# JosefAlbers/Phi-3-Vision-MLX

Measured on AMD Instinct MI355X. Metric: decode tokens/sec through generate()'s loop (reference-defined; bare graph replays: device_rate) + prefill ms, Phi-3-Vision bf16 1-image VQA, higher is better.
Workload: dtype bf16; 1 GPU; Phi-3-Vision single 336x336 image VQA (BASELINE configs[1]); 17 crops, 2509 image tokens + 22 text tokens, prompt 2531, B=1 per GPU, greedy, EOS suppressed; parallelism=batch-sharded replicas x1, batch_per_gpu=1, tiny=False

## Files before the change

include/p3v.h:

```cpp
#ifndef P3V_H
#define P3V_H
#include <stdint.h>

#ifdef __cplusplus
extern "C" {
#endif

#define P3V_VERSION 600
#define P3V_OK 0
#define P3V_ERR_ARG (-22)
#define P3V_ERR_LAUNCH (-5)
#define P3V_ERR_UNSUPPORTED (-95)
#define P3V_ERR_HIP (-14)

typedef struct {
  int cu_count, lds_per_cu, wave_size, clock_khz, mem_clock_khz, mem_bus_bits;
  int64_t hbm_bytes;
  char arch[32];
} p3v_props_t;

int p3v_version(void);
int p3v_device_props(int device, p3v_props_t* out );
const char* p3v_strerror(int code);

// ... 152 lines not shown
                 int h_crops, int w_crops, int grid , int C, void* stream);

int p3v_argmax(const uint16_t* logits, int32_t* out, int rows, int n, int64_t row_stride, void* stream);
int p3v_log_softmax(const uint16_t* x, uint16_t* y, int rows, int n, void* stream);
int p3v_topk(const uint16_t* x, int32_t* idx_out, int rows, int n, int k, int64_t row_stride, void* stream);

typedef struct {
  const uint16_t* x; const uint32_t* W; const uint32_t* sb; void* out;
  const uint16_t* resid; const uint16_t* norm_w; float norm_eps;
  int M, N, K;
  int epilogue;
} p3v_gemv_q4_args_t;
int p3v_gemv_q4(const p3v_gemv_q4_args_t* args , void* stream);
int p3v_dequant_q4(const uint32_t* w4, const uint32_t* sb, uint16_t* out_bf16, int rows, int K, void* stream);

int p3v_resample_u8(const uint8_t* in, uint8_t* out, int outer, int in_len, int out_len, int inner,
                    const int32_t* coeffs, const int32_t* bounds, int ksize, void* stream);
int p3v_hd_preprocess(const uint8_t* resized, int rh, int rw, int top, int hp, int portrait, const double* lut,
                      const float* hw, const int32_t* hi, const float* ww, const int32_t* wi, float* pixel_values,
                      int n_slots, void* stream);

int p3v_lora_down(const uint16_t* x, const float* lora_a, float* t, int M, int K, int r, void* stream);
int p3v_lora_up(const uint16_t* y, const float* t, const float* lora_b, float scale, int epilogue,
                const uint16_t* resid, uint16_t* out, int M, int N, int r, void* stream);

#define P3V_LORA_SLICE_K 256
typedef struct {
  const float* lora_a;
  const float* lora_b;
  int32_t rank;
// ... 15 lines not shown
                   int n_zero, void* stream);
int p3v_step_end(const uint16_t* logits, int32_t* next_tok, int32_t* tok, int32_t* history, int32_t* d_step,
                 int32_t* d_past, int32_t* ticket, int B, int n, int max_steps, void* stream);

#define P3V_GEMV_STEP_MAX_WG 1024
#define P3V_GEMV_STEP_WS_BYTES (P3V_GEMV_STEP_MAX_WG * 8 + 9 * 128)
typedef struct {
  const int32_t* tok; const uint16_t* embed_table; int vocab; uint16_t* x_out;
  const float* cos_t; const float* sin_t; float* cos_out; float* sin_out; int tab_t, half_dim;
  int32_t* next_tok; int32_t* tok_out; int32_t* history; int32_t* d_step; int32_t* ticket; float* amax_ws; int max_steps;
  int32_t* d_past;
} p3v_gemv_step_t;
int p3v_gemv_step(const p3v_gemv_args_t* args , const p3v_gemv_step_t* step , void* stream);
int p3v_gemv_fp8_step(const p3v_gemv_fp8_args_t* args , const p3v_gemv_step_t* step , void* stream);
int p3v_gemv_q4_step(const p3v_gemv_q4_args_t* args , const p3v_gemv_step_t* step , void* stream);

typedef struct {
  float temperature;
  int32_t top_k;
  float top_p;
  uint32_t seed_lo, seed_hi;
  int32_t counter;
} p3v_sample_row_t;
int p3v_sample(const uint16_t* logits, int64_t row_stride, p3v_sample_row_t* rows_params, int32_t* out, int rows, int n,
               void* stream);
int p3v_sample_step_end(const uint16_t* logits, p3v_sample_row_t* rows_params, int32_t* next_tok, int32_t* tok,
                        int32_t* history, int32_t* d_step, int32_t* d_past, int32_t* ticket, int B, int n, int max_steps,
                        void* stream);

#define P3V_LOGPROBS_MAX 8
// ... 60 lines not shown
```

phi-3-vision-mlx_amd/_lib.py:

```python
import ctypes as C
import os

_HERE = os.path.dirname(os.path.abspath(__file__))
LIB_PATH = os.environ.get("P3V_LIB") or os.path.join(_HERE, "libp3v.so")

P3V_OK = 0
(EPI_NONE, EPI_BIAS, EPI_BIAS_QGELU, EPI_BIAS_GELU, EPI_BIAS_RESID_F32, EPI_RESID_BF16, EPI_SILU_MUL, EPI_PATCH,
 EPI_F32) = range(9)
DECODE_MAX_L = 16

vp, i32, i64, f32 = C.c_void_p, C.c_int, C.c_int64, C.c_float


class Props(C.Structure):
    _fields_ = [("cu_count", i32), ("lds_per_cu", i32), ("wave_size", i32), ("clock_khz", i32),
                ("mem_clock_khz", i32), ("mem_bus_bits", i32), ("hbm_bytes", i64), ("arch", C.c_char * 32)]


class GemmArgs(C.Structure):
    _fields_ = [("A", vp), ("W", vp), ("out", vp), ("bias", vp), ("resid", vp), ("pos", vp),
                ("M", i32), ("N", i32), ("K", i32), ("lda", i32), ("ldw", i32), ("ldo", i32),
                ("epilogue", i32), ("patches_per_img", i32), ("ws", vp), ("ws_bytes", i64)]


# ... 125 lines not shown
    "p3v_kv_quantize_mlx4": (i32, [vp, vp, vp, vp, vp, vp, i32, i32, i32, i32, vp, vp, vp, i32, i32, i32, i32, i32, vp]),
    "p3v_attention_decode_q8": (i32, [C.POINTER(AttnDecQ8Args), vp]),
    "p3v_attention_decode_q8_can_fuse_oproj": (i32, [i32, i32, i32, i32, i32, i32, i32, i32]),
    "p3v_stage_rope": (i32, [vp, vp, i32, vp, vp, vp, i32, i32, i32, i32, vp]),
    "p3v_attention_ws_bytes": (i64, [i32, i32, i32, i32, i32]),
    "p3v_im2col_patches": (i32, [vp, vp, i32, i32, i32, i32, vp]),
    "p3v_clip_cls_rows": (i32, [vp, vp, vp, i32, i32, i32, vp]),
    "p3v_hd_merge": (i32, [vp, vp, vp, vp, i32, i32, i32, i32, vp]),
    "p3v_argmax": (i32, [vp, vp, i32, i32, i64, vp]),
    "p3v_log_softmax": (i32, [vp, vp, i32, i32, vp]),
    "p3v_topk": (i32, [vp, vp, i32, i32, i32, i64, vp]),
    "p3v_add_i32": (i32, [vp, i32, i32, vp]),
    "p3v_store_token": (i32, [vp, vp, vp, vp, i32, i32, vp]),
    "p3v_gemv_q4": (i32, [vp, vp]),
    "p3v_dequant_q4": (i32, [vp, vp, vp, i32, i32, vp]),
    "p3v_resample_u8": (i32, [vp, vp, i32, i32, i32, i32, vp, vp, i32, vp]),
    "p3v_hd_preprocess": (i32, [vp, i32, i32, i32, i32, i32, vp, vp, vp, vp, vp, vp, i32, vp]),
    "p3v_lora_down": (i32, [vp, vp, vp, i32, i32, i32, vp]),
    "p3v_lora_up": (i32, [vp, vp, vp, f32, i32, vp, vp, i32, i32, i32, vp]),
    "p3v_lora_rows_slices": (i32, [i32]),
    "p3v_lora_down_rows": (i32, [vp, vp, f32, vp, vp, vp, i32, i32, i32, i32, vp]),
    "p3v_lora_up_rows": (i32, [vp, vp, vp, vp, i32, vp, vp, i32, i32, i32, i32, i32, vp]),
    "p3v_step_begin": (i32, [vp, vp, vp, vp, vp, vp, vp, vp, i32, i32, i32, i32, i32, vp, i32, vp]),
    "p3v_step_end": (i32, [vp, vp, vp, vp, vp, vp, vp, i32, i32, i32, vp]),
    "p3v_sample": (i32, [vp, i64, vp, vp, i32, i32, vp]),
    "p3v_sample_step_end": (i32, [vp, vp, vp, vp, vp, vp, vp, vp, i32, i32, i32, vp]),
    "p3v_logprobs": (i32, [vp, i64, vp, vp, vp, i32, i32, vp]),
    "p3v_logprobs_step": (i32, [vp, vp, vp, vp, vp, i32, i32, i32, vp]),
    "p3v_spec_begin": (i32, [vp, vp, vp, vp, vp, vp, vp, vp, i32, i32, i32, i32, i32, vp]),
    "p3v_spec_end": (i32, [vp, C.POINTER(SpecState), i32, i32, vp]),
# ... 39 lines not shown
```

phi-3-vision-mlx_amd/model.py:

```python
import math
import copy
import os

import numpy as np
import torch

from . import ops
from .config import head_dim, is_vision, rope_scaling_factor
from .weights import Q4Weight, mlx_quantize, q4_repack
from .ops import (BF16, EPI_BIAS, EPI_BIAS_GELU, EPI_BIAS_QGELU, EPI_BIAS_RESID_F32, EPI_NONE, EPI_PATCH,
                  EPI_RESID_BF16, EPI_SILU_MUL, F32, I32)

import functools
import weakref


def _on_device(fn):
    @functools.wraps(fn)
    def wrapped(self, *a, **kw):
        with torch.cuda.device(self.device):
            return fn(self, *a, **kw)
    return wrapped


# ... 131 lines not shown
        self._bank_keep = []
        self._rows_cur = None
        self.serving = os.environ.get("P3V_SHARED_GPU", "0") == "1"
        self.epoch = 0
        self._prefill_graphs = {}
        self._prefill_seen = {}
        self._states = weakref.WeakSet()
        self.fp8_act = bool(getattr(cfg, "fp8_activations", True)) and os.environ.get("P3V_FP8_PREFILL", "mfma") != "dequant"
        if getattr(cfg, "quantized_fp8", False):
            self._quantize_decoder_fp8()
        if getattr(cfg, "quantized_int4", False):
            self._quantize_decoder_q4()
        if self.w4 and not hasattr(self, "_deq"):
            n_max = max(v[0].shape[0] * v[0].shape[1] * 8 for v in self.w4.values())
            self._deq = torch.empty(n_max, dtype=BF16, device=self.device)
        if self.vision:
            self._prep_vision()

    def _quantize_decoder_fp8(self):
        names = [k for k in self.w if k == "lm_head.weight" or (k.startswith("model.layers.") and k.endswith("_proj.weight"))]
        for k in names:
            self.w8[k] = ops.quantize_fp8_rows(self.w.pop(k))
        n_max = max(v[0].shape[0] * v[0].shape[1] for v in self.w8.values())
        self._deq = torch.empty(n_max, dtype=BF16, device=self.device)

    def set_adapters(self, adapters):
        if adapters and self._bank:
            raise ValueError("this model carries an adapter bank (set_adapter_bank): detach it before set_adapters -- one or the other")
        self._set_adapters(adapters)

    @_on_device
    def _set_adapters(self, adapters):
        for k, (a, b, _) in adapters.items():
            shape = self._weight_shape(k)
            if tuple(a.shape[:1]) != (shape[1],) or tuple(b.shape[1:]) != (shape[0],):
                raise ValueError(f"LoRA shapes {tuple(a.shape)} x {tuple(b.shape)} do not fit {k} {tuple(shape)}")
        self.adapters = {k: (a.to(self.device, F32).contiguous(), b.to(self.device, F32).contiguous(), float(s))
                         for k, (a, b, s) in adapters.items()}
        self.epoch += 1
# ... 114 lines not shown
        M, K, N, r = x.shape[0], x.shape[1], b.shape[1], a.shape[1]
        hbuf, y, t = self._lora_scratch(M, [("h", (M, K), BF16), ("y", (M, N), BF16), ("t", (M, r), F32)])
        if norm_w is not None:
            x = ops.rmsnorm(x, norm_w, self.cfg.rms_norm_eps, out=hbuf)
        self._proj_frozen(x, key, EPI_NONE, None, None, y, None)
        ops.lora_down(x, a, out=t)
        return ops.lora_up(y, t, b, scale, epilogue, resid=resid, out=out)

    def _proj_frozen(self, x, key, epilogue=EPI_NONE, resid=None, norm_w=None, out=None, h=None):
        eps = self.cfg.rms_norm_eps
        M, K = x.shape
        q, q4 = self.w8.get(key), self.w4.get(key)
        skinny = M <= 8 or (M <= ops.GEMV_MAX_M and K % 512 == 0)
        if skinny and M > 8 and q is None and q4 is None and K % 64 == 0 and self.w[key].shape[0] % 64 == 0:
            skinny = False
        if q4 is not None and M == 1 and K in (3072, 8192):
            return ops.gemv_q4(x, q4[0], q4[1], epilogue, resid=resid, norm_w=norm_w, norm_eps=eps, out=out)
        if (q4 is not None and 2 <= M <= 16 and K in (3072, 8192) and os.environ.get("P3V_Q4_ROWS", "1") != "0"
                and (q4[0].shape[0] // (2 if epilogue == EPI_SILU_MUL else 1)) % 16 == 0):
            if norm_w is not None and (M > 8 or os.environ.get("P3V_Q4_ROWS8_NORM", "1") == "0"):
                x, norm_w = ops.rmsnorm(x, norm_w, eps, out=h), None
            return ops.gemv_q4(x, q4[0], q4[1], epilogue, resid=resid, norm_w=norm_w, norm_eps=eps, out=out)
        if q is not None and skinny and K in (3072, 8192):
            return ops.gemv_fp8(x, q[0], q[1], epilogue, resid=resid, norm_w=norm_w, norm_eps=eps, out=out)
        if q is not None and not skinny and self.fp8_act and ops.gemm_fp8_ok(M, q[0].shape[0], K, epilogue):
            a8, sa = ops.quant_fp8_rows(x, norm_w, eps)
            return ops.gemm_fp8(a8, sa, q[0], q[1], epilogue, resid=resid, out=out)
        if q4 is not None:
            w = ops.dequant_q4(q4[0], q4[1], out=self._deq[:q4[0].numel() * 8].view(q4[0].shape[0], q4[0].shape[1] * 8))
        elif q is not None:
# ... 396 lines not shown
        for i in range(cfg.num_hidden_layers):
            p = f"model.layers.{i}."
            fused_qkv = False
            k_w = p + "self_attn.qkv_proj.weight"
            if (not decode and n_beam == 1 and k_w in w and k_w not in self.adapters and k_w not in self._bank and not mlx4_first
                    and (M >= 1024 or M <= 256) and os.environ.get("P3V_QKV_FUSE", "1") != "0"):
                kd, vd = (st.k_tmp, st.v_tmp) if st.quantized else (st.k[i], st.v[i])
                if not (st.quantized and past > 0 and not st.fresh_rows):
                    hn = h if normed_in else ops.rmsnorm(x, w[p + "input_layernorm.weight"], eps, out=h)
                    normed_in = True
                    fused_qkv = ops.gemm_qkv(hn, w[k_w], st.cos, st.sin, q, kd, vd, B, L, nh, nkv, hd, past, st.Tp, True, st.T, 1,
                                             q_scale=scale * ops.Q_PRESCALE)
            if i == 0 and step_begin is not None:
                sb = step_begin
                w_fold = w.get(k_w) if k_w in w else (self.w8.get(k_w) or self.w4.get(k_w))
                if not (w_fold is not None and k_w not in self.adapters and k_w not in self._bank and os.environ.get("P3V_STEP_FOLD", "1") != "0"
                        and ops.gemv_step_begin(sb["tok"], sb["table"], x, st.cos, st.sin, d_past, sb["cos_o"], sb["sin_o"],
                                                w_fold, w[p + "input_layernorm.weight"], eps, qkv)):
                    ops.step_begin(sb["tok"], sb["table"], x, st.cos, st.sin, d_past, sb["cos_o"], sb["sin_o"])
                    self._proj(x, k_w, norm_w=w[p + "input_layernorm.weight"], out=qkv, h=h)
            elif not fused_qkv:
                if normed_in:
                    self._proj(h, p + "self_attn.qkv_proj.weight", out=qkv)
                else:
                    self._proj(x, p + "self_attn.qkv_proj.weight", norm_w=w[p + "input_layernorm.weight"], out=qkv, h=h)
            o_i = o
            if fuse_o:
                o_i, o_other = (bufs["o_f"], bufs["o_f2"]) if i % 2 == 0 else (bufs["o_f2"], bufs["o_f"])
            if st.quantized:
                if decode:
# ... 82 lines not shown
        g["bufs"] = self._plan(st, B, 1, fuse_o=not st.slots, captured=True)
        g["amax_ws"] = torch.zeros((ops.L.GEMV_STEP_WS_BYTES // 4,), dtype=F32, device=dev)
        g["d_past"].fill_(st.offset)
        g["gemm_ws"] = {}
        g["graph"] = self._capture(lambda: self._decode_step(st, g), g["gemm_ws"])
        g["d_step"].zero_()
        return g

    def _decode_step(self, st, g, sampled=False, logprobs=False):
        cfg, w, bufs, head = self.cfg, self.w, g["bufs"], "lm_head.weight"
        self._layers(g["x"], st, st.B, 1, 0, 1, bufs=bufs, d_past=g["d_past"],
                     step_begin=dict(tok=g["tok"], table=w["model.embed_tokens.weight"], cos_o=bufs["rope_cos"], sin_o=bufs["rope_sin"]))
        end = (g["next_tok"], g["tok"], g["history"], g["d_step"], g["d_past"], g["ticket"])
        if not sampled:
            w_fold = w.get(head) if head in w else (self.w8.get(head) or self.w4.get(head))
            if (w_fold is not None and head not in self.adapters and os.environ.get("P3V_STEP_FOLD", "1") != "0"
                    and ops.gemv_step_end(g["x"], w_fold, w["model.norm.weight"], cfg.rms_norm_eps, g["logits"], *end, g["amax_ws"])):
                return self._logprobs_tail(st, g) if logprobs else None
        self._proj(g["x"], head, norm_w=w["model.norm.weight"], out=g["logits"], h=bufs["h"])
        if sampled:
            ops.sample_step_end(g["logits"], st.sample_rows, *end)
        else:
            ops.step_end(g["logits"], *end)
        if logprobs:
            self._logprobs_tail(st, g)

    def _logprobs_tail(self, st, g):
        ops.logprobs_step(g["logits"], g["next_tok"], st.logprob_want, g["d_step"], g["records"])

    def _replay(self, token, cache, which):
# ... 336 lines not shown
```

phi-3-vision-mlx_amd/ops.py:

```python
import contextlib
import ctypes as C

import numpy as np
import torch

from . import _lib as L
from ._lib import (EPI_BIAS, EPI_BIAS_GELU, EPI_BIAS_QGELU, EPI_BIAS_RESID_F32, EPI_F32, EPI_NONE,
                   EPI_PATCH, EPI_RESID_BF16, EPI_SILU_MUL)

BF16, F32, I32 = torch.bfloat16, torch.float32, torch.int32


def _stream():
    return torch.cuda.current_stream().cuda_stream


def _p(t):
    return 0 if t is None else t.data_ptr()


def _chk(t, dtype, name):
    if not t.is_cuda:
        raise RuntimeError(f"{name}: expected a device tensor (the hot path has no CPU fallback)")
    if t.dtype != dtype:
# ... 217 lines not shown
    M, K = x.shape
    N = w4.shape[0] // 2 if epilogue == EPI_SILU_MUL else w4.shape[0]
    if out is None:
        out = torch.empty((M, N), dtype=F32 if epilogue == EPI_F32 else BF16, device=x.device)
    args = L.GemvQ4Args(_p(x), _p(w4), _p(sb), _p(out), _p(resid), _p(norm_w), float(norm_eps), M, N, K, epilogue)
    L.check(L.lib().p3v_gemv_q4(C.byref(args), _stream()), "gemv_q4")
    return out


def dequant_q4(w4, sb, out=None):
    _chk(w4, I32, "w4"), _chk(sb, I32, "sb")
    N, K = w4.shape[0], w4.shape[1] * 8
    if out is None:
        out = torch.empty((N, K), dtype=BF16, device=w4.device)
    L.check(L.lib().p3v_dequant_q4(_p(w4), _p(sb), _p(out), N, K, _stream()), "dequant_q4")
    return out


def quantize_fp8_rows(w):
    wf = w.float()
    scale = (wf.abs().amax(dim=1) / 448.0).clamp_min(1e-12)
    w8 = (wf / scale[:, None]).to(torch.float8_e4m3fn).view(torch.uint8).contiguous()
    return w8, scale.contiguous()


def gemv_fp8(x, w8, w_scale, epilogue=EPI_NONE, resid=None, norm_w=None, norm_eps=0.0, out=None):
    _chk(x, BF16, "x"), _chk(w8, torch.uint8, "w8"), _chk(w_scale, F32, "w_scale")
    M, K = x.shape
    N = w8.shape[0] // 2 if epilogue == EPI_SILU_MUL else w8.shape[0]
    if out is None:
# ... 260 lines not shown
def gemv_step_begin(tok, table, x_out, cos_t, sin_t, d_past, cos_out, sin_out, w, norm_w, norm_eps, out):
    _chk(table, BF16, "table"), _chk(x_out, BF16, "x_out"), _chk(tok, I32, "tok")
    B, tab_t, half = tok.numel(), cos_t.shape[-2], cos_t.shape[-1]
    st = L.GemvStep(_p(tok), _p(table), table.shape[0], _p(x_out), _p(cos_t), _p(sin_t), _p(cos_out), _p(sin_out), tab_t, half,
                    None, None, None, None, None, None, 0, _p(d_past))
    if isinstance(w, tuple) and w[0].dtype == I32:
        w4, sb = w
        _chk(sb, I32, "sb")
        args = L.GemvQ4Args(None, _p(w4), _p(sb), _p(out), None, _p(norm_w), float(norm_eps), B, w4.shape[0], w4.shape[1] * 8, EPI_NONE)
        rc = L.lib().p3v_gemv_q4_step(C.byref(args), C.byref(st), _stream())
    elif isinstance(w, tuple):
        w8, ws = w
        _chk(w8, torch.uint8, "w8"), _chk(ws, F32, "w_scale")
        args = L.GemvF8Args(None, _p(w8), _p(ws), _p(out), None, _p(norm_w), float(norm_eps), B, w8.shape[0], w8.shape[1], EPI_NONE)
        rc = L.lib().p3v_gemv_fp8_step(C.byref(args), C.byref(st), _stream())
    else:
        _chk(w, BF16, "w")
        args = L.GemvArgs(None, _p(w), _p(out), None, _p(norm_w), float(norm_eps), B, w.shape[0], w.shape[1], EPI_NONE)
        rc = L.lib().p3v_gemv_step(C.byref(args), C.byref(st), _stream())
    if rc == L.ERR_UNSUPPORTED:
        return False
    L.check(rc, "gemv_step(begin)")
    return True


def gemv_step_end(x, w, norm_w, norm_eps, out, next_tok, tok, history, d_step, d_past, ticket, amax_ws):
    _chk(x, BF16, "x"), _chk(out, BF16, "out")
    if amax_ws.numel() * amax_ws.element_size() < L.GEMV_STEP_WS_BYTES:
        raise ValueError("gemv_step_end: amax_ws smaller than P3V_GEMV_STEP_WS_BYTES")
    M, K = x.shape
    st = L.GemvStep(None, None, 0, None, None, None, None, None, 0, 0,
                    _p(next_tok), _p(tok), _p(history), _p(d_step), _p(ticket), _p(amax_ws), history.shape[1], _p(d_past))
    if isinstance(w, tuple) and w[0].dtype == I32:
        w4, sb = w
        _chk(sb, I32, "sb")
        args = L.GemvQ4Args(_p(x), _p(w4), _p(sb), _p(out), None, _p(norm_w), float(norm_eps), M, w4.shape[0], K, EPI_NONE)
        rc = L.lib().p3v_gemv_q4_step(C.byref(args), C.byref(st), _stream())
    elif isinstance(w, tuple):
        w8, ws = w
        _chk(w8, torch.uint8, "w8"), _chk(ws, F32, "w_scale")
        args = L.GemvF8Args(_p(x), _p(w8), _p(ws), _p(out), None, _p(norm_w), float(norm_eps), M, w8.shape[0], K, EPI_NONE)
        rc = L.lib().p3v_gemv_fp8_step(C.byref(args), C.byref(st), _stream())
    else:
        _chk(w, BF16, "w")
        args = L.GemvArgs(_p(x), _p(w), _p(out), None, _p(norm_w), float(norm_eps), M, w.shape[0], K, EPI_NONE)
        rc = L.lib().p3v_gemv_step(C.byref(args), C.byref(st), _stream())
    if rc == L.ERR_UNSUPPORTED:
        return False
    L.check(rc, "gemv_step(end)")
    return True


def add_i32(x, delta):
    L.check(L.lib().p3v_add_i32(_p(x), x.numel(), int(delta), _stream()), "add_i32")


def step_begin(tok, table, x_out, cos_t, sin_t, d_past, cos_out, sin_out, zero_buf=None):
# ... 160 lines not shown
```

Measured before the change: 535.0 tokens/s.

## Add lossless 13-bit packed bf16 weight format and GEMV for decode

Adds a per-row lossless repacking of bf16 weights into 13 bits per element: sign plane, 7-bit mantissa plus the low exponent bit, 4-bit exponent nibble, and a per-row exponent base. A matching GEMV and fused step kernels decode the weights in registers with packed integer ops and bf16 dot2. Decode is bound by weight bandwidth, so reading about 13/16 of the bytes should shorten each matvec. Rows whose exponent range exceeds 31 or that contain inf, NaN or subnormal values fall back to plain bf16. The cost is extra ALU work per weight, a one-time pack, and extra memory for the packed copy.

Result: no change. 534.6 tokens/s, median of 2 (-0.1%).

```diff
diff --git a/include/p3v.h b/include/p3v.h
--- a/include/p3v.h
+++ b/include/p3v.h
@@ -190,6 +190,17 @@
 int p3v_gemv_q4(const p3v_gemv_q4_args_t* args , void* stream);
 int p3v_dequant_q4(const uint32_t* w4, const uint32_t* sb, uint16_t* out_bf16, int rows, int K, void* stream);
 
+typedef struct {
+  const uint16_t* x; const void* W; void* out;
+  const uint16_t* resid; const uint16_t* norm_w; float norm_eps;
+  int M, N, K;
+  int epilogue;
+} p3v_gemv_pk_args_t;
+int64_t p3v_pack13_bytes(int rows, int K);
+int p3v_pack13(const uint16_t* W, int rows, int K, void* packed, int32_t* bad_rows, void* stream);
+int p3v_unpack13(const void* packed, uint16_t* W_out, int rows, int K, void* stream);
+int p3v_gemv_pk(const p3v_gemv_pk_args_t* args , void* stream);
+
 int p3v_resample_u8(const uint8_t* in, uint8_t* out, int outer, int in_len, int out_len, int inner,
                     const int32_t* coeffs, const int32_t* bounds, int ksize, void* stream);
 int p3v_hd_preprocess(const uint8_t* resized, int rh, int rw, int top, int hp, int portrait, const double* lut,
@@ -235,6 +246,7 @@
 int p3v_gemv_step(const p3v_gemv_args_t* args , const p3v_gemv_step_t* step , void* stream);
 int p3v_gemv_fp8_step(const p3v_gemv_fp8_args_t* args , const p3v_gemv_step_t* step , void* stream);
 int p3v_gemv_q4_step(const p3v_gemv_q4_args_t* args , const p3v_gemv_step_t* step , void* stream);
+int p3v_gemv_pk_step(const p3v_gemv_pk_args_t* args , const p3v_gemv_step_t* step , void* stream);
 
 typedef struct {
   float temperature;
diff --git a/phi-3-vision-mlx_amd/_lib.py b/phi-3-vision-mlx_amd/_lib.py
--- a/phi-3-vision-mlx_amd/_lib.py
+++ b/phi-3-vision-mlx_amd/_lib.py
@@ -163,6 +163,11 @@
     "p3v_store_token": (i32, [vp, vp, vp, vp, i32, i32, vp]),
     "p3v_gemv_q4": (i32, [vp, vp]),
     "p3v_dequant_q4": (i32, [vp, vp, vp, i32, i32, vp]),
+    "p3v_pack13_bytes": (i64, [i32, i32]),
+    "p3v_pack13": (i32, [vp, i32, i32, vp, vp, vp]),
+    "p3v_unpack13": (i32, [vp, vp, i32, i32, vp]),
+    "p3v_gemv_pk": (i32, [C.POINTER(GemvArgs), vp]),
+    "p3v_gemv_pk_step": (i32, [C.POINTER(GemvArgs), C.POINTER(GemvStep), vp]),
     "p3v_resample_u8": (i32, [vp, vp, i32, i32, i32, i32, vp, vp, i32, vp]),
     "p3v_hd_preprocess": (i32, [vp, i32, i32, i32, i32, i32, vp, vp, vp, vp, vp, vp, i32, vp]),
     "p3v_lora_down": (i32, [vp, vp, vp, i32, i32, i32, vp]),
diff --git a/phi-3-vision-mlx_amd/csrc/p3v_dot_pk.h b/phi-3-vision-mlx_amd/csrc/p3v_dot_pk.h
--- /dev/null
+++ b/phi-3-vision-mlx_amd/csrc/p3v_dot_pk.h
@@ -0,0 +1,58 @@
+#pragma once
+#include "p3v_common.h"
+
+template <int NST, int CH>
+struct PkRow {
+  static_assert(CH % 2 == 0 && CH <= 8, "chunks per stage: pairs of chunks per byte-plane load, at most two sign dwords");
+  static constexpr int K = NST * CH * 512;
+  static constexpr int SW = (CH + 3) / 4;
+  static constexpr int NIB_OFF = K, SGN_OFF = K + K / 2, HDR_OFF = SGN_OFF + NST * 64 * SW * 4, BYTES = HDR_OFF + 16;
+  __host__ __device__ static constexpr int sm_off(int s, int j, int l) { return ((s * (CH / 2) + j / 2) * 64 + l) * 16 + (j & 1) * 8; }
+  __host__ __device__ static constexpr int nib_off(int s, int j, int l) {
+    return NIB_OFF + s * CH * 256 + (j < (CH / 4) * 4 ? (j / 4) * 1024 + l * 16 + (j & 3) * 4 : (CH / 4) * 1024 + l * 8 + (j & 1) * 4);
+  }
+  __host__ __device__ static constexpr int sgn_off(int s, int q, int l) { return SGN_OFF + ((s * 64 + l) * SW + q) * 4; }
+};
+
+typedef unsigned short pk_u16x2_t __attribute__((ext_vector_type(2)));
+typedef __bf16 pk_pair_t __attribute__((ext_vector_type(2)));
+typedef __bf16 pk_oct_t __attribute__((ext_vector_type(8)));
+
+__device__ __forceinline__ uint32_t pk_pair_bits(uint32_t x, uint32_t e2) {
+#if defined(__HIP_DEVICE_COMPILE__)
+  const uint32_t one = 0x00010001u;
+  uint32_t t, nz, y;
+  asm("v_pk_lshlrev_b16 %0, %1, %2" : "=v"(t) : "s"(one), "v"(x));
+  asm("v_pk_min_u16 %0, %1, %2" : "=v"(nz) : "v"(t), "s"(one));
+  asm("v_pk_mad_u16 %0, %1, %2, %3" : "=v"(y) : "v"(nz), "v"(e2), "v"(x));
+  return y;
+#else
+  const uint32_t nz = ((x & 0x7fffu) ? 1u : 0u) | ((x & 0x7fff0000u) ? 0x10000u : 0u);
+  return x + nz * (e2 & 0xffffu);
+#endif
+}
+
+template <int JJ>
+__device__ __forceinline__ u32x4_t pk_decode8(uint32_t b0, uint32_t b1, uint32_t nb, uint32_t sd, uint32_t e2) {
+  const uint32_t h0 = (nb & 0x0F0F0F0Fu) | ((sd << (2 * JJ)) & 0x80808080u);
+  const uint32_t h1 = ((nb >> 4) & 0x0F0F0F0Fu) | ((sd << (2 * JJ + 1)) & 0x80808080u);
+  u32x4_t p;
+  p[0] = pk_pair_bits(__builtin_amdgcn_perm(h0, b0, 0x05010400u), e2);
+  p[1] = pk_pair_bits(__builtin_amdgcn_perm(h0, b0, 0x07030602u), e2);
+  p[2] = pk_pair_bits(__builtin_amdgcn_perm(h1, b1, 0x05010400u), e2);
+  p[3] = pk_pair_bits(__builtin_amdgcn_perm(h1, b1, 0x07030602u), e2);
+  return p;
+}
+
+template <int JJ>
+__device__ __forceinline__ float dot8_pk(uint32_t b0, uint32_t b1, uint32_t nb, uint32_t sd, uint32_t e2, u32x4_t x, float acc) {
+  const pk_oct_t xv = __builtin_bit_cast(pk_oct_t, x);
+  const u32x4_t p = pk_decode8<JJ>(b0, b1, nb, sd, e2);
+  uint32_t q0 = p[0], q1 = p[1], q2 = p[2], q3 = p[3];
+  asm("" : "+v"(q0), "+v"(q1), "+v"(q2), "+v"(q3));
+  acc = __builtin_amdgcn_fdot2_f32_bf16(__builtin_bit_cast(pk_pair_t, q0), __builtin_shufflevector(xv, xv, 0, 1), acc, false);
+  acc = __builtin_amdgcn_fdot2_f32_bf16(__builtin_bit_cast(pk_pair_t, q1), __builtin_shufflevector(xv, xv, 2, 3), acc, false);
+  acc = __builtin_amdgcn_fdot2_f32_bf16(__builtin_bit_cast(pk_pair_t, q2), __builtin_shufflevector(xv, xv, 4, 5), acc, false);
+  acc = __builtin_amdgcn_fdot2_f32_bf16(__builtin_bit_cast(pk_pair_t, q3), __builtin_shufflevector(xv, xv, 6, 7), acc, false);
+  return acc;
+}
diff --git a/phi-3-vision-mlx_amd/csrc/p3v_gemv_pk.hip b/phi-3-vision-mlx_amd/csrc/p3v_gemv_pk.hip
--- /dev/null
+++ b/phi-3-vision-mlx_amd/csrc/p3v_gemv_pk.hip
@@ -0,0 +1,348 @@
+#include <stdlib.h>
+
+#include <type_traits>
+
+#include "p3v_common.h"
+#include "p3v_dot_pk.h"
+#include "p3v_gemv3_body.h"
+
+template <int NST, int CH>
+__global__ void __launch_bounds__(256) k_pack13(const bf16_t* __restrict__ W, unsigned char* __restrict__ out, int32_t* __restrict__ bad_rows) {
+  typedef PkRow<NST, CH> R;
+  constexpr int ITEMS = NST * R::SW * 64;
+  static_assert(ITEMS <= 256, "one work item per thread");
+  __shared__ int s_min, s_max, s_bad;
+  const int tid = threadIdx.x, row = blockIdx.x;
+  if (tid == 0) { s_min = 256; s_max = 0; s_bad = 0; }
+  __syncthreads();
+  const int l = tid & 63, q = (tid >> 6) % R::SW, s = (tid >> 6) / R::SW;
+  const bool live = tid < ITEMS;
+  u32x4_t w[4];
+  int emin = 256, emax = 0, bad = 0;
+#pragma unroll
+  for (int jj = 0; jj < 4; ++jj) {
+    const int j = 4 * q + jj;
+    const bool on = live && j < CH;
+    w[jj] = on ? ((const u32x4_t*)(W + (size_t)row * R::K))[(s * CH + j) * 64 + l] : (u32x4_t){0, 0, 0, 0};
+#pragma unroll
+    for (int i = 0; i < 8; ++i) {
+      const uint32_t v = (w[jj][i >> 1] >> (16 * (i & 1))) & 0xffffu, e = (v >> 7) & 0xffu, m = v & 0x7fu;
+      if (e == 255u || (e == 0u && m != 0u)) bad = 1;
+      if (e != 0u) { emin = min(emin, (int)e); emax = max(emax, (int)e); }
+    }
+  }
+  atomicMin(&s_min, emin);
+  atomicMax(&s_max, emax);
+  if (bad) atomicOr(&s_bad, 1);
+  __syncthreads();
+  const int e_lo = s_max == 0 ? 0 : s_min - 1;
+  unsigned char* rec = out + (size_t)row * R::BYTES;
+  if (tid == 0) {
+    if (s_bad || s_max - e_lo > 31) atomicAdd(bad_rows, 1);
+    *(u32x4_t*)(rec + R::HDR_OFF) = (u32x4_t){((uint32_t)e_lo << 7) * 0x00010001u, 0u, 0u, 0u};
+  }
+  if (!live) return;
+  uint32_t sd = 0;
+#pragma unroll
+  for (int jj = 0; jj < 4; ++jj) {
+    const int j = 4 * q + jj;
+    if (j < CH) {
+      uint32_t b[2] = {0, 0}, nb = 0;
+#pragma unroll
+      for (int i = 0; i < 8; ++i) {
+        const uint32_t v = (w[jj][i >> 1] >> (16 * (i & 1))) & 0xffffu, e = (v >> 7) & 0xffu, m = v & 0x7fu;
+        const uint32_t f = (v & 0x7fffu) ? (e - (uint32_t)e_lo) & 31u : 0u;
+        const int h = i >> 2, t = i & 3;
+        b[h] |= (((f & 1u) << 7) | m) << (8 * t);
+        nb |= (f >> 1) << (8 * t + 4 * h);
+        sd |= (v >> 15) << (8 * t + 7 - 2 * jj - h);
+      }
+      *(u32x2_t*)(rec + R::sm_off(s, j, l)) = (u32x2_t){b[0], b[1]};
+      *(uint32_t*)(rec + R::nib_off(s, j, l)) = nb;
+    }
+  }
+  *(uint32_t*)(rec + R::sgn_off(s, q, l)) = sd;
+}
+
+template <int NST, int CH>
+__global__ void __launch_bounds__(256) k_unpack13(const unsigned char* __restrict__ in, bf16_t* __restrict__ W) {
+  typedef PkRow<NST, CH> R;
+  const int row = blockIdx.x, l = threadIdx.x & 63;
+  const unsigned char* rec = in + (size_t)row * R::BYTES;
+  const uint32_t e2 = *(const uint32_t*)(rec + R::HDR_OFF);
+  for (int it = threadIdx.x >> 6; it < NST * CH; it += 4) {
+    const int s = it / CH, j = it % CH;
+    const u32x2_t b = *(const u32x2_t*)(rec + R::sm_off(s, j, l));
+    const uint32_t nb = *(const uint32_t*)(rec + R::nib_off(s, j, l)), sd = *(const uint32_t*)(rec + R::sgn_off(s, j / 4, l));
+    u32x4_t p;
+    switch (j & 3) {
+      case 0: p = pk_decode8<0>(b[0], b[1], nb, sd, e2); break;
+      case 1: p = pk_decode8<1>(b[0], b[1], nb, sd, e2); break;
+      case 2: p = pk_decode8<2>(b[0], b[1], nb, sd, e2); break;
+      default: p = pk_decode8<3>(b[0], b[1], nb, sd, e2); break;
+    }
+    ((u32x4_t*)(W + (size_t)row * R::K))[(s * CH + j) * 64 + l] = p;
+  }
+}
+
+extern "C" int64_t p3v_pack13_bytes(int rows, int K) {
+  if (rows <= 0) return 0;
+  if (K == 3072) return (int64_t)rows * PkRow<1, 6>::BYTES;
+  if (K == 8192) return (int64_t)rows * PkRow<4, 4>::BYTES;
+  return 0;
+}
+
+extern "C" int p3v_pack13(const uint16_t* W, int rows, int K, void* packed, int32_t* bad_rows, void* stream) {
+  if (!W || !packed || !bad_rows || rows <= 0 || K <= 0) return P3V_ERR_ARG;
+  if (((uintptr_t)W | (uintptr_t)packed) & 15) return P3V_ERR_ARG;
+  if (K != 3072 && K != 8192) return P3V_ERR_UNSUPPORTED;
+  hipStream_t s = (hipStream_t)stream;
+  if (K == 3072) hipLaunchKernelGGL((k_pack13<1, 6>), dim3(rows), dim3(256), 0, s, W, (unsigned char*)packed, bad_rows);
+  else hipLaunchKernelGGL((k_pack13<4, 4>), dim3(rows), dim3(256), 0, s, W, (unsigned char*)packed, bad_rows);
+  P3V_CHECK_LAUNCH();
+  return P3V_OK;
+}
+
+extern "C" int p3v_unpack13(const void* packed, uint16_t* W, int rows, int K, void* stream) {
+  if (!W || !packed || rows <= 0 || K <= 0) return P3V_ERR_ARG;
+  if (((uintptr_t)W | (uintptr_t)packed) & 15) return P3V_ERR_ARG;
+  if (K != 3072 && K != 8192) return P3V_ERR_UNSUPPORTED;
+  hipStream_t s = (hipStream_t)stream;
+  if (K == 3072) hipLaunchKernelGGL((k_unpack13<1, 6>), dim3(rows), dim3(256), 0, s, (const unsigned char*)packed, W);
+  else hipLaunchKernelGGL((k_unpack13<4, 4>), dim3(rows), dim3(256), 0, s, (const unsigned char*)packed, W);
+  P3V_CHECK_LAUNCH();
+  return P3V_OK;
+}
+
+struct GemvPkP {
+  const bf16_t* x; const unsigned char* W; void* out; const bf16_t* resid; const bf16_t* norm_w;
+  float eps;
+  int M, N, K, epi, units;
+};
+typedef std::integral_constant<int, 0> PC0;
+typedef std::integral_constant<int, 1> PC1;
+
+template <int NST, int CH, int STEP>
+__device__ __forceinline__ void gemv3_pk_body(const GemvPkP& p, int units_per_wave, int wpw, unsigned char* smem, float* red, const GemvStepP* sp) {
+  typedef PkRow<NST, CH> R;
+  constexpr int CHUNKS = NST * CH * 64;
+  constexpr int XC = (CHUNKS + 255) / 256;
+  constexpr int NB4 = CH / 4, SW = R::SW;
+  u32x4_t* xs = (u32x4_t*)smem;
+  const int tid = threadIdx.x, lane = tid & 63, wave = tid >> 6, bx = blockIdx.x;
+  const bool silu = p.epi == P3V_EPI_SILU_MUL, has_res = p.epi == P3V_EPI_RESID_BF16;
+  const int u_begin = wave < wpw ? min(p.units, (bx * wpw + wave) * units_per_wave) : p.units;
+  const int u_end = min(p.units, u_begin + units_per_wave);
+  const int n_st = (u_end - u_begin) * NST;
+
+  u32x4_t xv[XC], gv[XC];
+  const bf16_t* xrow[1] = {p.x};
+  if (STEP == STEP_BEGIN) {
+    int id = sp->tok[0];
+    id = id < 0 ? 0 : (id >= sp->vocab ? sp->vocab - 1 : id);
+    xrow[0] = sp->table + (size_t)id * (CHUNKS * 8);
+  }
+#pragma unroll
+  for (int k = 0; k < XC; ++k) {
+    const int c = min(tid + k * 256, CHUNKS - 1);
+    xv[k] = ((const u32x4_t*)xrow[0])[c];
+    gv[k] = p.norm_w ? ((const u32x4_t*)p.norm_w)[c] : (u32x4_t){0, 0, 0, 0};
+  }
+
+  u32x4_t bbuf[2][2][CH / 2];
+  uint32_t nbuf[2][2][CH], sbuf[2][2][SW], ebuf[2][2];
+  uint32_t rbuf[2];
+  auto issue = [&](int gs, auto bufc) {
+    constexpr int buf = decltype(bufc)::value;
+    const int u = min(u_begin + gs / NST, p.units - 1), s = gs % NST;
+    const int r0 = silu ? u : 2 * u, r1 = silu ? u + p.N : min(2 * u + 1, p.N - 1);
+#pragma unroll
+    for (int h = 0; h < 2; ++h) {
+      const unsigned char* rec = p.W + (size_t)(h ? r1 : r0) * R::BYTES;
+      const u32x4_t* bp = (const u32x4_t*)rec + s * (CH / 2) * 64 + lane;
+#pragma unroll
+      for (int i = 0; i < CH / 2; ++i) bbuf[buf][h][i] = __builtin_nontemporal_load(bp + i * 64);
+      const unsigned char* np = rec + R::NIB_OFF + s * CH * 256;
+#pragma unroll
+      for (int g = 0; g < NB4; ++g) {
+        const u32x4_t v = __builtin_nontemporal_load((const u32x4_t*)(np + g * 1024) + lane);
+        nbuf[buf][h][4 * g] = v[0]; nbuf[buf][h][4 * g + 1] = v[1]; nbuf[buf][h][4 * g + 2] = v[2]; nbuf[buf][h][4 * g + 3] = v[3];
+      }
+      if constexpr (CH % 4 == 2) {
+        const u32x2_t v = __builtin_nontemporal_load((const u32x2_t*)(np + NB4 * 1024) + lane);
+        nbuf[buf][h][CH - 2] = v[0]; nbuf[buf][h][CH - 1] = v[1];
+      }
+      const unsigned char* gp = rec + R::SGN_OFF;
+      if constexpr (SW == 2) {
+        const u32x2_t v = __builtin_nontemporal_load((const u32x2_t*)gp + s * 64 + lane);
+        sbuf[buf][h][0] = v[0]; sbuf[buf][h][1] = v[1];
+      } else {
+        sbuf[buf][h][0] = __builtin_nontemporal_load((const uint32_t*)gp + s * 64 + lane);
+      }
+      ebuf[buf][h] = *(const uint32_t*)(rec + R::HDR_OFF);
+    }
+    rbuf[buf] = !has_res ? 0u : *(const uint32_t*)(p.resid + 2 * u);
+  };
+  if (n_st > 0) issue(0, PC0{});
+
+  float r = 1.f;
+  if (p.norm_w) {
+    float ss = 0.f;
+#pragma unroll
+    for (int k = 0; k < XC; ++k) {
+      if (tid + k * 256 < CHUNKS) {
+#pragma unroll
+        for (int j = 0; j < 4; ++j) { const float a = bf16lo(xv[k][j]), b = bf16hi(xv[k][j]); ss += a * a + b * b; }
+      }
+    }
+    ss = wave_sum(ss);
+    if (lane == 0) red[wave] = ss;
+    asm volatile("s_waitcnt lgkmcnt(0)" ::: "memory");
+    __builtin_amdgcn_s_barrier();
+    r = rsqrtf(((red[0] + red[1]) + (red[2] + red[3])) / (float)(CHUNKS * 8) + p.eps);
+  }
+#pragma unroll
+  for (int k = 0; k < XC; ++k) {
+    const int c = tid + k * 256;
+    if (c < CHUNKS) {
+      u32x4_t o = xv[k];
+      if (p.norm_w) {
+#pragma unroll
+        for (int j = 0; j < 4; ++j) o[j] = rms_pair(xv[k][j], r, gv[k][j]);
+      }
+      xs[c] = o;
+    }
+  }
+  asm volatile("s_waitcnt lgkmcnt(0)" ::: "memory");
+  __builtin_amdgcn_s_barrier();
+
+  float a0 = 0.f, a1 = 0.f;
+  ArgMaxVI best[1] = {ArgMaxVI{-INFINITY, 0x7fffffff}};
+  auto chunk = [&](auto bufc, auto jc, int s) {
+    constexpr int buf = decltype(bufc)::value, j = decltype(jc)::value;
+    const u32x4_t xa = xs[(s * CH + j) * 64 + lane];
+    a0 = dot8_pk<(j & 3)>(bbuf[buf][0][j / 2][(j & 1) * 2], bbuf[buf][0][j / 2][(j & 1) * 2 + 1], nbuf[buf][0][j], sbuf[buf][0][j / 4], ebuf[buf][0], xa, a0);
+    a1 = dot8_pk<(j & 3)>(bbuf[buf][1][j / 2][(j & 1) * 2], bbuf[buf][1][j / 2][(j & 1) * 2 + 1], nbuf[buf][1][j], sbuf[buf][1][j / 4], ebuf[buf][1], xa, a1);
+  };
+  auto compute = [&](int gs, auto bufc) {
+    constexpr int buf = decltype(bufc)::value;
+    const int s = gs % NST;
+    chunk(bufc, std::integral_constant<int, 0>{}, s);
+    chunk(bufc, std::integral_constant<int, 1>{}, s);
+    if constexpr (CH > 2) { chunk(bufc, std::integral_constant<int, 2>{}, s); chunk(bufc, std::integral_constant<int, 3>{}, s); }
+    if constexpr (CH > 4) { chunk(bufc, std::integral_constant<int, 4>{}, s); chunk(bufc, std::integral_constant<int, 5>{}, s); }
+    if constexpr (CH > 6) { chunk(bufc, std::integral_constant<int, 6>{}, s); chunk(bufc, std::integral_constant<int, 7>{}, s); }
+    if (s == NST - 1) {
+      const int u = u_begin + gs / NST;
+      a0 = wave_sum(a0);
+      a1 = wave_sum(a1);
+      if (lane == 0) {
+        if (silu) {
+          const float g = bf16_round(a0), up = bf16_round(a1);
+          const float sg = bf16_round(g * bf16_round(1.f / (1.f + __expf(-g))));
+          ((bf16_t*)p.out)[u] = f32_to_bf16(sg * up);
+        } else if (p.epi == P3V_EPI_F32) {
+          ((float*)p.out)[2 * u] = a0;
+          ((float*)p.out)[2 * u + 1] = a1;
+        } else {
+          float v0 = a0, v1 = a1;
+          if (has_res) { v0 = bf16lo(rbuf[buf]) + bf16_round(v0); v1 = bf16hi(rbuf[buf]) + bf16_round(v1); }
+          *(uint32_t*)((bf16_t*)p.out + 2 * u) = pack_bf16x2(v0, v1);
+          if (STEP == STEP_END) {
+            amax_take(best[0], bf16_round(v0), 2 * u);
+            if (2 * u + 1 < p.N) amax_take(best[0], bf16_round(v1), 2 * u + 1);
+          }
+        }
+      }
+      a0 = a1 = 0.f;
+    }
+  };
+  int gs = 0;
+  while (gs + 2 < n_st) {
+    issue(gs + 1, PC1{}); compute(gs, PC0{});
+    issue(gs + 2, PC0{}); compute(gs + 1, PC1{});
+    gs += 2;
+  }
+  if (gs + 1 < n_st) {
+    issue(gs + 1, PC1{}); compute(gs, PC0{}); compute(gs + 1, PC1{});
+  } else if (gs < n_st) {
+    compute(gs, PC0{});
+  }
+  if (STEP == STEP_BEGIN && bx == 0) gemv_step_begin_tail<1>(sp, xrow, 1, CHUNKS, tid);
+  if (STEP == STEP_END) gemv_step_end_tail<1>(sp, best, 1, bx, tid);
+}
+
+template <int NST, int CH>
+__global__ void __launch_bounds__(256) k_gemv3_pk(GemvPkP p, int units_per_wave, int wpw) {
+  extern __shared__ __attribute__((aligned(16))) unsigned char smem[];
+  __shared__ float red[4];
+  gemv3_pk_body<NST, CH, STEP_NONE>(p, units_per_wave, wpw, smem, red, nullptr);
+}
+
+template <int NST, int CH, int STEP>
+__global__ void __launch_bounds__(256) k_gemv3_pk_step(GemvPkP p, int units_per_wave, int wpw, GemvStepP sp) {
+  extern __shared__ __attribute__((aligned(16))) unsigned char smem[];
+  __shared__ float red[4];
+  gemv3_pk_body<NST, CH, STEP>(p, units_per_wave, wpw, smem, red, &sp);
+}
+
+template <int NST, int CH, int STEP = STEP_NONE>
+static int launch_gemv3_pk(const GemvPkP& p, hipStream_t s, const GemvStepP* sp = nullptr) {
+  static int n_cu = 0;
+  if (!n_cu) {
+    int dev = 0;
+    hipDeviceProp_t pr;
+    if (hipGetDevice(&dev) != hipSuccess || hipGetDeviceProperties(&pr, dev) != hipSuccess) return P3V_ERR_HIP;
+    n_cu = pr.multiProcessorCount;
+  }
+  const int wpc = p3v_tuning().gemv_wpc;
+  int upw = p3v_cdiv(p.units, n_cu * wpc);
+  if (upw < 1) upw = 1;
+  const int waves = p3v_cdiv(p.units, upw);
+  const int wpw = p3v_gemv_wpw(waves, n_cu, p3v_tuning().gemv_wpw);
+  const size_t lds = (size_t)p.K * 2;
+  if constexpr (STEP != STEP_NONE) {
+    if (p3v_cdiv(waves, wpw) > P3V_GEMV_STEP_MAX_WG) return P3V_ERR_UNSUPPORTED;
+    hipLaunchKernelGGL((k_gemv3_pk_step<NST, CH, STEP>), dim3(p3v_cdiv(waves, wpw)), dim3(256), lds, s, p, upw, wpw, *sp);
+  } else {
+    hipLaunchKernelGGL((k_gemv3_pk<NST, CH>), dim3(p3v_cdiv(waves, wpw)), dim3(256), lds, s, p, upw, wpw);
+  }
+  P3V_CHECK_LAUNCH();
+  return P3V_OK;
+}
+
+extern "C" int p3v_gemv_pk(const p3v_gemv_pk_args_t* a, void* stream) {
+  if (!a || !a->x || !a->W || !a->out) return P3V_ERR_ARG;
+  if (a->M <= 0 || a->N <= 0 || a->K <= 0) return P3V_ERR_ARG;
+  if (a->M != 1 || a->N % 2 || (a->K != 3072 && a->K != 8192)) return P3V_ERR_UNSUPPORTED;
+  if (a->epilogue != P3V_EPI_NONE && a->epilogue != P3V_EPI_RESID_BF16 && a->epilogue != P3V_EPI_SILU_MUL && a->epilogue != P3V_EPI_F32)
+    return P3V_ERR_UNSUPPORTED;
+  if (a->epilogue == P3V_EPI_RESID_BF16 && !a->resid) return P3V_ERR_ARG;
+  if (((uintptr_t)a->x | (uintptr_t)a->W | (uintptr_t)a->norm_w) & 15) return P3V_ERR_ARG;
+  const GemvPkP p = {a->x, (const unsigned char*)a->W, a->out, a->resid, a->norm_w, a->norm_eps, a->M, a->N, a->K, a->epilogue,
+                     a->epilogue == P3V_EPI_SILU_MUL ? a->N : a->N / 2};
+  hipStream_t s = (hipStream_t)stream;
+  return a->K == 3072 ? launch_gemv3_pk<1, 6>(p, s) : launch_gemv3_pk<4, 4>(p, s);
+}
+
+extern "C" int p3v_gemv_pk_step(const p3v_gemv_pk_args_t* a, const p3v_gemv_step_t* st, void* stream) {
+  if (!a || !st || !a->W || !a->out) return P3V_ERR_ARG;
+  const bool begin = st->tok != nullptr, end = st->next_tok != nullptr;
+  if (begin == end) return P3V_ERR_ARG;
+  if (a->M <= 0 || a->N <= 0 || a->K <= 0) return P3V_ERR_ARG;
+  if (a->M != 1 || a->N % 2 || (a->K != 3072 && a->K != 8192) || a->epilogue != P3V_EPI_NONE) return P3V_ERR_UNSUPPORTED;
+  if (((uintptr_t)a->W | (uintptr_t)a->norm_w) & 15) return P3V_ERR_ARG;
+  if (begin) {
+    if (!st->embed_table || !st->x_out || !st->cos_t || !st->sin_t || !st->d_past || !st->cos_out || !st->sin_out || st->vocab <= 0) return P3V_ERR_ARG;
+    if (((uintptr_t)st->embed_table | (uintptr_t)st->x_out) & 15) return P3V_ERR_ARG;
+  } else {
+    if (!a->x || !st->tok_out || !st->history || !st->d_step || !st->d_past || !st->ticket || !st->amax_ws) return P3V_ERR_ARG;
+    if ((uintptr_t)st->amax_ws & 7) return P3V_ERR_ARG;
+  }
+  const GemvPkP p = {a->x, (const unsigned char*)a->W, a->out, a->resid, a->norm_w, a->norm_eps, a->M, a->N, a->K, a->epilogue, a->N / 2};
+  const GemvStepP sp = {st->tok, st->embed_table, st->vocab, st->x_out, st->cos_t, st->sin_t, st->d_past, st->cos_out, st->sin_out, st->tab_t,
+                        st->half_dim, st->next_tok, st->tok_out, st->history, st->d_step, st->d_past, st->ticket, st->amax_ws, st->max_steps};
+  hipStream_t s = (hipStream_t)stream;
+  if (a->K == 3072) return begin ? launch_gemv3_pk<1, 6, STEP_BEGIN>(p, s, &sp) : launch_gemv3_pk<1, 6, STEP_END>(p, s, &sp);
+  return begin ? launch_gemv3_pk<4, 4, STEP_BEGIN>(p, s, &sp) : launch_gemv3_pk<4, 4, STEP_END>(p, s, &sp);
+}
diff --git a/phi-3-vision-mlx_amd/model.py b/phi-3-vision-mlx_amd/model.py
--- a/phi-3-vision-mlx_amd/model.py
+++ b/phi-3-vision-mlx_amd/model.py
@@ -169,6 +169,9 @@
         if self.w4 and not hasattr(self, "_deq"):
             n_max = max(v[0].shape[0] * v[0].shape[1] * 8 for v in self.w4.values())
             self._deq = torch.empty(n_max, dtype=BF16, device=self.device)
+        self.wpk = {}
+        if os.environ.get("P3V_PACKED_WEIGHTS", "0") == "1" and not self.w8 and not self.w4:
+            self._pack_decoder()
         if self.vision:
             self._prep_vision()
 
@@ -178,6 +181,23 @@
             self.w8[k] = ops.quantize_fp8_rows(self.w.pop(k))
         n_max = max(v[0].shape[0] * v[0].shape[1] for v in self.w8.values())
         self._deq = torch.empty(n_max, dtype=BF16, device=self.device)
+
+    @_on_device
+    def _pack_decoder(self):
+        names = [k for k in self.w if k == "lm_head.weight" or (k.startswith("model.layers.") and k.endswith(
+            ("self_attn.qkv_proj.weight", "mlp.gate_up_proj.weight", "mlp.down_proj.weight")))]
+        names = [k for k in names if self.w[k].shape[0] % 2 == 0 and ops.pack13_bytes(*self.w[k].shape)]
+        if not names:
+            return
+        packed = [ops.pack13(self.w[k]) for k in names]
+        bad = torch.cat([b for _, b in packed]).cpu()
+        self.wpk = {k: (wp, self.w[k], self.w[k]._version) for k, (wp, _), n in zip(names, packed, bad.tolist()) if n == 0}
+
+    def _packed(self, key):
+        e = self.wpk.get(key)
+        if e is None or self.w.get(key) is not e[1] or e[1]._version != e[2]:
+            return None
+        return e[0]
 
     def set_adapters(self, adapters):
         if adapters and self._bank:
@@ -322,6 +342,8 @@
         skinny = M <= 8 or (M <= ops.GEMV_MAX_M and K % 512 == 0)
         if skinny and M > 8 and q is None and q4 is None and K % 64 == 0 and self.w[key].shape[0] % 64 == 0:
             skinny = False
+        if M == 1 and self._packed(key) is not None:
+            return ops.gemv_pk(x, self._packed(key), epilogue, resid=resid, norm_w=norm_w, norm_eps=eps, out=out)
         if q4 is not None and M == 1 and K in (3072, 8192):
             return ops.gemv_q4(x, q4[0], q4[1], epilogue, resid=resid, norm_w=norm_w, norm_eps=eps, out=out)
         if (q4 is not None and 2 <= M <= 16 and K in (3072, 8192) and os.environ.get("P3V_Q4_ROWS", "1") != "0"
@@ -748,6 +770,8 @@
             if i == 0 and step_begin is not None:
                 sb = step_begin
                 w_fold = w.get(k_w) if k_w in w else (self.w8.get(k_w) or self.w4.get(k_w))
+                if B == 1 and self._packed(k_w) is not None:
+                    w_fold = self._packed(k_w)
                 if not (w_fold is not None and k_w not in self.adapters and k_w not in self._bank and os.environ.get("P3V_STEP_FOLD", "1") != "0"
                         and ops.gemv_step_begin(sb["tok"], sb["table"], x, st.cos, st.sin, d_past, sb["cos_o"], sb["sin_o"],
                                                 w_fold, w[p + "input_layernorm.weight"], eps, qkv)):
@@ -860,6 +884,8 @@
         end = (g["next_tok"], g["tok"], g["history"], g["d_step"], g["d_past"], g["ticket"])
         if not sampled:
             w_fold = w.get(head) if head in w else (self.w8.get(head) or self.w4.get(head))
+            if st.B == 1 and self._packed(head) is not None:
+                w_fold = self._packed(head)
             if (w_fold is not None and head not in self.adapters and os.environ.get("P3V_STEP_FOLD", "1") != "0"
                     and ops.gemv_step_end(g["x"], w_fold, w["model.norm.weight"], cfg.rms_norm_eps, g["logits"], *end, g["amax_ws"])):
                 return self._logprobs_tail(st, g) if logprobs else None
diff --git a/phi-3-vision-mlx_amd/ops.py b/phi-3-vision-mlx_amd/ops.py
--- a/phi-3-vision-mlx_amd/ops.py
+++ b/phi-3-vision-mlx_amd/ops.py
@@ -255,6 +255,42 @@
     if out is None:
         out = torch.empty((N, K), dtype=BF16, device=w4.device)
     L.check(L.lib().p3v_dequant_q4(_p(w4), _p(sb), _p(out), N, K, _stream()), "dequant_q4")
+    return out
+
+
+def pack13_bytes(rows, K):
+    return int(L.lib().p3v_pack13_bytes(int(rows), int(K)))
+
+
+def pack13(w, out=None):
+    _chk(w, BF16, "w")
+    N, K = w.shape
+    nb = pack13_bytes(N, K)
+    if nb == 0:
+        raise ValueError(f"pack13: K = {K} is not supported")
+    out = torch.empty((N, nb // N), dtype=torch.uint8, device=w.device) if out is None else _chk(out, torch.uint8, "out")
+    if out.numel() != nb:
+        raise ValueError(f"pack13: out holds {out.numel()} bytes, {nb} needed")
+    bad = torch.zeros((1,), dtype=I32, device=w.device)
+    L.check(L.lib().p3v_pack13(_p(w), N, K, _p(out), _p(bad), _stream()), "pack13")
+    return out, bad
+
+
+def unpack13(wp, K):
+    _chk(wp, torch.uint8, "wp")
+    out = torch.empty((wp.shape[0], K), dtype=BF16, device=wp.device)
+    L.check(L.lib().p3v_unpack13(_p(wp), _p(out), wp.shape[0], int(K), _stream()), "unpack13")
+    return out
+
+
+def gemv_pk(x, wp, epilogue=EPI_NONE, resid=None, norm_w=None, norm_eps=0.0, out=None):
+    _chk(x, BF16, "x"), _chk(wp, torch.uint8, "wp")
+    M, K = x.shape
+    N = wp.shape[0] // 2 if epilogue == EPI_SILU_MUL else wp.shape[0]
+    if out is None:
+        out = torch.empty((M, N), dtype=F32 if epilogue == EPI_F32 else BF16, device=x.device)
+    args = L.GemvArgs(_p(x), _p(wp), _p(out), _p(resid), _p(norm_w), float(norm_eps), M, N, K, epilogue)
+    L.check(L.lib().p3v_gemv_pk(C.byref(args), _stream()), "gemv_pk")
     return out
 
 
@@ -545,6 +581,10 @@
         _chk(w8, torch.uint8, "w8"), _chk(ws, F32, "w_scale")
         args = L.GemvF8Args(None, _p(w8), _p(ws), _p(out), None, _p(norm_w), float(norm_eps), B, w8.shape[0], w8.shape[1], EPI_NONE)
         rc = L.lib().p3v_gemv_fp8_step(C.byref(args), C.byref(st), _stream())
+    elif w.dtype == torch.uint8:
+        _chk(w, torch.uint8, "wp")
+        args = L.GemvArgs(None, _p(w), _p(out), None, _p(norm_w), float(norm_eps), B, w.shape[0], table.shape[1], EPI_NONE)
+        rc = L.lib().p3v_gemv_pk_step(C.byref(args), C.byref(st), _stream())
     else:
         _chk(w, BF16, "w")
         args = L.GemvArgs(None, _p(w), _p(out), None, _p(norm_w), float(norm_eps), B, w.shape[0], w.shape[1], EPI_NONE)
@@ -572,6 +612,10 @@
         _chk(w8, torch.uint8, "w8"), _chk(ws, F32, "w_scale")
         args = L.GemvF8Args(_p(x), _p(w8), _p(ws), _p(out), None, _p(norm_w), float(norm_eps), M, w8.shape[0], K, EPI_NONE)
         rc = L.lib().p3v_gemv_fp8_step(C.byref(args), C.byref(st), _stream())
+    elif w.dtype == torch.uint8:
+        _chk(w, torch.uint8, "wp")
+        args = L.GemvArgs(_p(x), _p(w), _p(out), None, _p(norm_w), float(norm_eps), M, w.shape[0], K, EPI_NONE)
+        rc = L.lib().p3v_gemv_pk_step(C.byref(args), C.byref(st), _stream())
     else:
         _chk(w, BF16, "w")
         args = L.GemvArgs(_p(x), _p(w), _p(out), None, _p(norm_w), float(norm_eps), M, w.shape[0], K, EPI_NONE)
diff --git a/phi-3-vision-mlx_amd/pack13.py b/phi-3-vision-mlx_amd/pack13.py
--- /dev/null
+++ b/phi-3-vision-mlx_amd/pack13.py
@@ -0,0 +1,74 @@
+import torch
+
+GEOMETRY = {3072: (1, 6), 8192: (4, 4)}
+
+
+def _bits(w):
+    if w.dtype == torch.bfloat16:
+        w = w.contiguous().view(torch.int16)
+    return w.to(torch.int32) & 0xFFFF
+
+
+def fields(w):
+    b = _bits(w)
+    s, e, m = b >> 15, (b >> 7) & 0xFF, b & 0x7F
+    nz = e != 0
+    bad = ((e == 255) | ((e == 0) & (m != 0))).any(dim=1)
+    emin = torch.where(nz, e, torch.full_like(e, 256)).amin(dim=1)
+    emax = e.amax(dim=1)
+    e_lo = torch.where(emax == 0, torch.zeros_like(emin), emin - 1)
+    f = torch.where((b & 0x7FFF) != 0, (e - e_lo[:, None]) & 31, torch.zeros_like(e))
+    return s, m, f, e_lo, ~bad & (emax - e_lo <= 31)
+
+
+def from_fields(s, m, f, e_lo):
+    e = torch.where(f != 0, e_lo[:, None] + f, torch.zeros_like(f))
+    b = (s << 15) | (e << 7) | m
+    return torch.where(b >= 32768, b - 65536, b).to(torch.int16).view(torch.bfloat16)
+
+
+def row_bytes(K):
+    nst, ch = GEOMETRY[K]
+    return K + K // 2 + nst * 64 * ((ch + 3) // 4) * 4 + 16
+
+
+def _index_maps(K):
+    nst, ch = GEOMETRY[K]
+    sw = (ch + 3) // 4
+    k = torch.arange(K)
+    c, i = k // 8, k % 8
+    lane, sj = c % 64, c // 64
+    s, j = sj // ch, sj % ch
+    h, t = i // 4, i % 4
+    sm = ((s * (ch // 2) + j // 2) * 64 + lane) * 16 + (j % 2) * 8 + i
+    full = (ch // 4) * 4
+    nib_dw = K + s * ch * 256 + torch.where(j < full, (j // 4) * 1024 + lane * 16 + (j % 4) * 4, (ch // 4) * 1024 + lane * 8 + (j % 2) * 4)
+    nib_bit = 8 * t + 4 * h
+    sgn_dw = K + K // 2 + ((s * 64 + lane) * sw + j // 4) * 4
+    sgn_bit = 8 * t + 7 - 2 * (j % 4) - h
+    return sm, nib_dw + nib_bit // 8, nib_bit % 8, sgn_dw + sgn_bit // 8, sgn_bit % 8
+
+
+def pack_rows(w):
+    rows, K = w.shape
+    s, m, f, e_lo, ok = fields(w)
+    sm, nb, nsh, sg, ssh = _index_maps(K)
+    rec = torch.zeros((rows, row_bytes(K)), dtype=torch.int32)
+    rec[:, sm] = (((f & 1) << 7) | m).to(torch.int32)
+    rec.index_add_(1, nb, ((f >> 1) << nsh).to(torch.int32))
+    rec.index_add_(1, sg, (s << ssh).to(torch.int32))
+    hdr = row_bytes(K) - 16
+    e2 = e_lo << 7
+    for i, v in enumerate((e2 & 0xFF, e2 >> 8, e2 & 0xFF, e2 >> 8)):
+        rec[:, hdr + i] = v
+    return rec.to(torch.uint8), int((~ok).sum())
+
+
+def unpack_rows(rec, K):
+    r = rec.to(torch.int32)
+    sm, nb, nsh, sg, ssh = _index_maps(K)
+    lo = r[:, sm]
+    hdr = row_bytes(K) - 16
+    e_lo = (r[:, hdr] | (r[:, hdr + 1] << 8)) >> 7
+    f = (((r[:, nb] >> nsh) & 15) << 1) | (lo >> 7)
+    return from_fields((r[:, sg] >> ssh) & 1, lo & 0x7F, f, e_lo)
```
